# xuekt98/BBDM

Measured on NVIDIA H100. Metric: denoising-steps/sec (UNet fwd) at 256^2 pixel-BBDM, higher is better.
Workload: dtype bf16x3 (split-bf16 tensor-core products, fp32 accumulate: fp32-class)

## Files before the change

### bbdm_b200/csrc/conv_umma.cu

```cuda
#include "tc_common.cuh"
#include <stdlib.h>

namespace bbdm {

constexpr int UM_BM = 128;
constexpr int UM_BK = 64;
constexpr int UM_THREADS = 384;
constexpr int UM_PRODUCER_REGS = 40, UM_CONSUMER_REGS = 232;
static_assert(128 * UM_PRODUCER_REGS + 256 * UM_CONSUMER_REGS <= 65536, "conv_umma: register split");
constexpr int UM_SLICES = 4;

struct ConvParams {
  int B, H, W, Cout;
  int TW, TH, TB, tiles_w, tiles_h, tiles_b, n_tiles;
  int kb_per_tap;
  int K1;
  int K2;
  int taps;
  int up2;
  int origin;
  int w_per_image;
  int kb_per_chunk;
  const float* bias; const float* bias2;
  const float* residual; int res_mode;
  float* out; __nv_bfloat16* out_hi; __nv_bfloat16* out_lo;
  int out_nchw_c;
  float* stats;
  unsigned long long* fault;
};

template <int BN>
struct UmmaCfg {
  static constexpr uint32_t A_BYTES = UM_BM * UM_BK * 2;
  static constexpr uint32_t W_BYTES = BN * UM_BK * 2;
  static constexpr uint32_t STAGE3 = 2 * A_BYTES + 2 * W_BYTES;
  static constexpr uint32_t STAGE1 = A_BYTES + W_BYTES;
  static constexpr uint32_t SMEM_BUDGET = 200 * 1024;
  static constexpr int STAGES3 = (SMEM_BUDGET / STAGE3) > 6 ? 6 : (SMEM_BUDGET / STAGE3);
  static constexpr int STAGES1 = (SMEM_BUDGET / STAGE1) > 8 ? 8 : (SMEM_BUDGET / STAGE1);
};

template <int BN, bool F16>
__device__ __forceinline__ void conv_mma(float* d, uint64_t da, uint64_t db) {
  if (F16) {
    if (BN == 128) wgmma_n128_f16<0>(d, da, db, 1u); else wgmma_n64_f16<0>(d, da, db, 1u);
  } else {
    if (BN == 128) wgmma_n128_bf16<0>(d, da, db, 1u); else wgmma_n64_bf16<0>(d, da, db, 1u);
  }
}

struct EpiTile {
  int nb, tw, th, tb, phase;
  int bb[2], hh[2], ww[2];
  bool valid[2];
  int64_t pix[2];
};

__device__ __forceinline__ EpiTile epi_tile(const ConvParams& p, int tile, int n_blocks, int warp, int lane) {
  EpiTile e;
  e.nb = tile % n_blocks;
  int mt = tile / n_blocks;
  e.phase = 0;
  if (p.up2) { e.phase = mt & 3; mt >>= 2; }
  e.tw = mt % p.tiles_w; mt /= p.tiles_w;
  e.th = mt % p.tiles_h;
  e.tb = mt / p.tiles_h;
  const int OH = p.up2 ? 2 * p.H : p.H, OW = p.up2 ? 2 * p.W : p.W;
#pragma unroll
  for (int ri = 0; ri < 2; ++ri) {
    const int row = 16 * warp + (lane >> 2) + 8 * ri;
    const int ws = e.tw * p.TW + row % p.TW;
    const int hs = e.th * p.TH + (row / p.TW) % p.TH;
    e.bb[ri] = e.tb * p.TB + row / (p.TW * p.TH);
    e.valid[ri] = ws < p.W && hs < p.H && e.bb[ri] < p.B;
    e.hh[ri] = p.up2 ? 2 * hs + (e.phase >> 1) : hs;
    e.ww[ri] = p.up2 ? 2 * ws + (e.phase & 1) : ws;
    e.pix[ri] = ((int64_t)e.bb[ri] * OH + e.hh[ri]) * OW + e.ww[ri];
  }
  return e;
}

template <int BN>
__device__ __forceinline__ void epi_slice(const ConvParams& p, const float* racc, EpiTile e, int s, int warp,
                                          int lane, float (*stats_s)[BN][2]) {
  constexpr int JS = BN / 8 / UM_SLICES;
  if (e.nb * BN + s * (BN / UM_SLICES) >= p.Cout) return;
  asm volatile("" : "+r"(e.nb), "+r"(e.bb[0]), "+r"(e.bb[1]), "+r"(e.hh[0]), "+r"(e.hh[1]), "+r"(e.ww[0]),
               "+r"(e.ww[1]), "+l"(e.pix[0]), "+l"(e.pix[1]));
  const int OH = p.up2 ? 2 * p.H : p.H, OW = p.up2 ? 2 * p.W : p.W;
  const int n0 = e.nb * BN + 2 * (lane & 3);
  float2 v[2][JS];
#pragma unroll
  for (int ri = 0; ri < 2; ++ri) {
#pragma unroll
    for (int j = 0; j < JS; ++j) {
      const int jj = JS * s + j;
      const int nc = n0 + 8 * jj;
      v[ri][j] = make_float2(racc[4 * jj + 2 * ri], racc[4 * jj + 2 * ri + 1]);
      if (p.bias) { const float2 b = *reinterpret_cast<const float2*>(p.bias + nc); v[ri][j].x += b.x; v[ri][j].y += b.y; }
      if (p.bias2) { const float2 b = *reinterpret_cast<const float2*>(p.bias2 + nc); v[ri][j].x += b.x; v[ri][j].y += b.y; }
    }
  }
  if (p.res_mode == BBDM_RES_SAME || p.res_mode == BBDM_RES_UP2) {
#pragma unroll
    for (int ri = 0; ri < 2; ++ri) {
      if (!e.valid[ri]) continue;
      const int64_t rpix = p.res_mode == BBDM_RES_SAME
                               ? e.pix[ri]
                               : ((int64_t)e.bb[ri] * (OH >> 1) + (e.hh[ri] >> 1)) * (OW >> 1) + (e.ww[ri] >> 1);
      const float* rp = p.residual + rpix * p.Cout + n0 + 8 * JS * s;
#pragma unroll
      for (int j = 0; j < JS; ++j) {
        const float2 t = *reinterpret_cast<const float2*>(rp + 8 * j);
        v[ri][j].x += t.x; v[ri][j].y += t.y;
      }
    }
  } else if (p.res_mode == BBDM_RES_DOWN2) {
    const int64_t W2 = (int64_t)OW * 2;
#pragma unroll
    for (int ri = 0; ri < 2; ++ri) {
      if (!e.valid[ri]) continue;
      const float* rp0 = p.residual + (((int64_t)e.bb[ri] * OH * 2 + e.hh[ri] * 2) * W2 + e.ww[ri] * 2) * p.Cout +
                         n0 + 8 * JS * s;
#pragma unroll
      for (int j = 0; j < JS; ++j) {
        const float* rp = rp0 + 8 * j;
        const float2 t0 = *reinterpret_cast<const float2*>(rp), t1 = *reinterpret_cast<const float2*>(rp + p.Cout);
        const float2 t2 = *reinterpret_cast<const float2*>(rp + W2 * p.Cout);
        const float2 t3 = *reinterpret_cast<const float2*>(rp + (W2 + 1) * p.Cout);
        v[ri][j].x += 0.25f * (((t0.x + t1.x) + t2.x) + t3.x);
        v[ri][j].y += 0.25f * (((t0.y + t1.y) + t2.y) + t3.y);
      }
    }
  }
  float ssum[2 * JS], ssq[2 * JS];
#pragma unroll
  for (int j = 0; j < 2 * JS; ++j) { ssum[j] = 0.f; ssq[j] = 0.f; }
#pragma unroll
  for (int ri = 0; ri < 2; ++ri) {
    if (!e.valid[ri]) continue;
    const int bb = e.bb[ri], hh = e.hh[ri], ww = e.ww[ri];
    const int64_t pix = e.pix[ri];
#pragma unroll
    for (int j = 0; j < JS; ++j) {
      const int nc = n0 + 8 * (JS * s + j);
      const float2 w = v[ri][j];
      if (p.out_nchw_c > 0) {
        if (nc < p.out_nchw_c) p.out[(((int64_t)bb * p.out_nchw_c + nc) * OH + hh) * OW + ww] = w.x;
        if (nc + 1 < p.out_nchw_c) p.out[(((int64_t)bb * p.out_nchw_c + nc + 1) * OH + hh) * OW + ww] = w.y;
      } else if (p.out) {
        *reinterpret_cast<float2*>(p.out + pix * p.Cout + nc) = w;
      }
      if (p.out_hi) {
        uint32_t h, l;
        split2x(w.x, w.y, h, l);
        *reinterpret_cast<uint32_t*>(p.out_hi + pix * p.Cout + nc) = h;
        *reinterpret_cast<uint32_t*>(p.out_lo + pix * p.Cout + nc) = l;
      }
      ssum[2 * j] += w.x; ssq[2 * j] += w.x * w.x;
      ssum[2 * j + 1] += w.y; ssq[2 * j + 1] += w.y * w.y;
    }
  }
  if (p.stats) {
#pragma unroll
    for (int j = 0; j < 2 * JS; ++j) {
#pragma unroll
      for (int off = 4; off < 32; off <<= 1) {
        ssum[j] += __shfl_xor_sync(0xffffffffu, ssum[j], off);
        ssq[j] += __shfl_xor_sync(0xffffffffu, ssq[j], off);
      }
    }
    if (lane < 4) {
#pragma unroll
      for (int j = 0; j < 2 * JS; ++j) {
        const int c = 8 * (JS * s + (j >> 1)) + 2 * lane + (j & 1);
        stats_s[warp][c][0] = ssum[j];
        stats_s[warp][c][1] = ssq[j];
      }
    }
  }
}

template <int BN>
__device__ __forceinline__ void epi_stats_out(const ConvParams& p, const EpiTile& e, float (*stats_s)[BN][2]) {
  if (!p.stats) return;
  asm volatile("bar.sync 1, 256;" ::: "memory");
  const int64_t tile_lin =
      (((int64_t)e.tb * p.tiles_w * p.tiles_h + e.th * p.tiles_w + e.tw) * (p.up2 ? 4 : 1) + e.phase) * 4;
  int i0 = threadIdx.x;
  asm volatile("" : "+r"(i0));
  for (int i = i0; i < 4 * BN; i += 256) {
    const int q = i / BN, c = i % BN;
    if (e.nb * BN + c >= p.Cout) continue;
    const float s = stats_s[2 * q][c][0] + stats_s[2 * q + 1][c][0];
    const float sq = stats_s[2 * q][c][1] + stats_s[2 * q + 1][c][1];
    *reinterpret_cast<float2*>(p.stats + ((tile_lin + q) * p.Cout + e.nb * BN + c) * 2) = make_float2(s, sq);
  }
  asm volatile("bar.sync 1, 256;" ::: "memory");
}

template <int BN>
__device__ __forceinline__ void epi_slices(const ConvParams& p, const float* racc, const EpiTile& e, int s_begin,
                                           int s_end, int warp, int lane, float (*stats_s)[BN][2]) {
#pragma unroll
  for (int s = 0; s < UM_SLICES; ++s)
    if (s >= s_begin && s < s_end) epi_slice<BN>(p, racc, e, s, warp, lane, stats_s);
}

template <int BN, int PASSES, bool F16>
__global__ void __launch_bounds__(UM_THREADS, 1)
conv_umma_kernel(const __grid_constant__ CUtensorMap map_a_hi, const __grid_constant__ CUtensorMap map_a_lo,
                 const __grid_constant__ CUtensorMap map_w_hi, const __grid_constant__ CUtensorMap map_w_lo,
                 const __grid_constant__ CUtensorMap map_a2_hi, const __grid_constant__ CUtensorMap map_a2_lo,
                 const __grid_constant__ CUtensorMap map_w2_hi, const __grid_constant__ CUtensorMap map_w2_lo,
                 const ConvParams p) {
  using Cfg = UmmaCfg<BN>;
  constexpr int STAGES = PASSES == 3 ? Cfg::STAGES3 : Cfg::STAGES1;
  constexpr uint32_t STAGE_BYTES = PASSES == 3 ? Cfg::STAGE3 : Cfg::STAGE1;
  constexpr uint32_t OFF_ALO = Cfg::A_BYTES;
  constexpr uint32_t OFF_WHI = PASSES == 3 ? 2 * Cfg::A_BYTES : Cfg::A_BYTES;
  constexpr uint32_t OFF_WLO = OFF_WHI + Cfg::W_BYTES;
  constexpr int NR = BN / 2;
  static_assert(STAGES >= 2, "need at least a double buffer");

  extern __shared__ uint8_t smem_raw[];
  __shared__ __align__(8) uint64_t bars[2 * 8];
  __shared__ int abort_s;
  __shared__ __align__(16) float stats_s[8][BN][2];

  const uint32_t tiles_base = (smem_u32(smem_raw) + 1023u) & ~1023u;
  const int warp = threadIdx.x >> 5, lane = threadIdx.x & 31;
  const uint32_t bar_full = smem_u32(&bars[0]);
  const uint32_t bar_empty = smem_u32(&bars[8]);
  volatile int* abort_flag = &abort_s;

  if (threadIdx.x == 0) {
    abort_s = 0;
    for (int i = 0; i < STAGES; ++i) { mbar_init(bar_full + 8 * i, 1); mbar_init(bar_empty + 8 * i, 8); }
    asm volatile("fence.mbarrier_init.release.cluster;" ::: "memory");
  }
  __syncthreads();

  const int n_blocks = (p.Cout + BN - 1) / BN;
  const int total_tiles = p.n_tiles * n_blocks * (p.up2 ? 4 : 1);
  const int KB = p.K1 + p.K2;

  if (warp >= 8) {
    setmaxnreg_dec<UM_PRODUCER_REGS>();
    if (warp == 8 && lane == 0) {
      int stage = 0;
      uint32_t phase_bit = 0;
      for (int tile = blockIdx.x; tile < total_tiles; tile += gridDim.x) {
        const int nb = tile % n_blocks;
        int mt = tile / n_blocks;
        int phase = 0;
        if (p.up2) { phase = mt & 3; mt >>= 2; }
        const int tw = mt % p.tiles_w; mt /= p.tiles_w;
        const int th = mt % p.tiles_h;
        const int tb = mt / p.tiles_h;
        const int w0 = tw * p.TW, h0 = th * p.TH, b0 = tb * p.TB, n0 = nb * BN;
        for (int kb = 0; kb < KB; ++kb) {
          mbar_wait(bar_empty + 8 * stage, phase_bit ^ 1, abort_flag, p.fault, 0xE0000000ull | (unsigned)kb);
          const uint32_t sbase = tiles_base + stage * STAGE_BYTES;
          const uint32_t full = bar_full + 8 * stage;
          mbar_expect_tx(full, STAGE_BYTES);
          if (kb < p.K1) {
            const int tap = kb / p.kb_per_tap, cb = kb - tap * p.kb_per_tap;
            int dy = 0, dx = 0, wtap = tap;
            if (p.up2) {
              const int r = tap >> 1, c = tap & 1;
              dy = (phase >> 1) ? r : r - 1;
              dx = (phase & 1) ? c : c - 1;
              wtap = phase * 4 + tap;
            } else if (p.taps == 9) { dy = tap / 3 - 1; dx = tap % 3 - 1; }
            else if (p.taps == 4) { dy = (tap >> 1) + p.origin; dx = (tap & 1) + p.origin; }
            else if (p.w_per_image) wtap = tb;
            tma_load_4d(sbase, &map_a_hi, full, cb * UM_BK, w0 + dx, h0 + dy, b0);
            if (PASSES == 3) tma_load_4d(sbase + OFF_ALO, &map_a_lo, full, cb * UM_BK, w0 + dx, h0 + dy, b0);
            tma_load_3d(sbase + OFF_WHI, &map_w_hi, full, cb * UM_BK, n0, wtap);
            if (PASSES == 3) tma_load_3d(sbase + OFF_WLO, &map_w_lo, full, cb * UM_BK, n0, wtap);
          } else {
            const int cb = kb - p.K1;
            tma_load_4d(sbase, &map_a2_hi, full, cb * UM_BK, w0, h0, b0);
            if (PASSES == 3) tma_load_4d(sbase + OFF_ALO, &map_a2_lo, full, cb * UM_BK, w0, h0, b0);
            tma_load_3d(sbase + OFF_WHI, &map_w2_hi, full, cb * UM_BK, n0, 0);
            if (PASSES == 3) tma_load_3d(sbase + OFF_WLO, &map_w2_lo, full, cb * UM_BK, n0, 0);
          }
          if (++stage == STAGES) { stage = 0; phase_bit ^= 1; }
        }
      }
    }
    return;
  }

  setmaxnreg_inc<UM_CONSUMER_REGS>();
  const int wg = warp >> 2;
  const uint32_t a_off = (uint32_t)wg * 64 * 128;
  int stage = 0;
  uint32_t phase_bit = 0;
  float racc[NR];
  EpiTile pend;
  bool pending = false;
  int slice = 0;
  for (int tile = blockIdx.x; tile < total_tiles; tile += gridDim.x) {
    for (int kb0 = 0; kb0 < KB; kb0 += p.kb_per_chunk) {
      const int kb1 = kb0 + p.kb_per_chunk < KB ? kb0 + p.kb_per_chunk : KB;
      float acc[NR];
#pragma unroll
      for (int j = 0; j < NR; ++j) acc[j] = 0.f;
      int prev = -1;
      for (int kb = kb0; kb < kb1; ++kb) {
        mbar_wait(bar_full + 8 * stage, phase_bit, abort_flag, p.fault, 0xF0000000ull | (unsigned)kb);
        const uint32_t sbase = tiles_base + stage * STAGE_BYTES;
        const uint64_t da_hi = make_sw128_desc(sbase + a_off);
        const uint64_t da_lo = make_sw128_desc(sbase + OFF_ALO + a_off);
        const uint64_t db_hi = make_sw128_desc(sbase + OFF_WHI);
        const uint64_t db_lo = make_sw128_desc(sbase + OFF_WLO);
        wgmma_fence();
#pragma unroll
        for (int k = 0; k < UM_BK / 16; ++k) {
          const uint64_t ko = (uint64_t)(k * 32 >> 4);
          if (PASSES == 3) {
            conv_mma<BN, F16>(acc, da_lo + ko, db_hi + ko);
            conv_mma<BN, F16>(acc, da_hi + ko, db_lo + ko);
          }
          conv_mma<BN, F16>(acc, da_hi + ko, db_hi + ko);
        }
        wgmma_commit();
        wgmma_wait<1>();
        if (prev >= 0 && lane == 0) mbar_arrive(bar_empty + 8 * prev);
        prev = stage;
        if (++stage == STAGES) { stage = 0; phase_bit ^= 1; }
        if (pending) {
          const int s_end = kb + 1 < kb1 ? slice + 1 : UM_SLICES;
          epi_slices<BN>(p, racc, pend, slice, s_end, warp, lane, stats_s);
          slice = s_end;
        }
      }
      if (pending) {
        epi_stats_out<BN>(p, pend, stats_s);
        pending = false;
      }
      wgmma_wait<0>();
      reg_fence<NR>(acc);
      if (lane == 0) mbar_arrive(bar_empty + 8 * prev);
      if (kb0 == 0) {
#pragma unroll
        for (int j = 0; j < NR; ++j) racc[j] = 0.f + acc[j];
      } else {
#pragma unroll
        for (int j = 0; j < NR; ++j) racc[j] += acc[j];
      }
    }
    pend = epi_tile(p, tile, n_blocks, warp, lane);
    pending = true;
    slice = 0;
  }
  if (pending) {
    epi_slices<BN>(p, racc, pend, 0, UM_SLICES, warp, lane, stats_s);
    epi_stats_out<BN>(p, pend, stats_s);
  }
}

static int make_act_map(CUtensorMap* m, const void* ptr, int B, int H, int W, int C, int TW, int TH, int TB,
                        bool f16) {
  EncodeTiledFn enc = get_encode();
  BBDM_REQUIRE(enc != nullptr, "cuTensorMapEncodeTiled entry point not available");
  cuuint64_t dims[4] = {(cuuint64_t)C, (cuuint64_t)W, (cuuint64_t)H, (cuuint64_t)B};
  cuuint64_t strides[3] = {(cuuint64_t)C * 2, (cuuint64_t)W * C * 2, (cuuint64_t)H * W * C * 2};
  cuuint32_t box[4] = {(cuuint32_t)UM_BK, (cuuint32_t)TW, (cuuint32_t)TH, (cuuint32_t)TB};
  cuuint32_t es[4] = {1, 1, 1, 1};
  CUresult r = enc(m, f16 ? CU_TENSOR_MAP_DATA_TYPE_FLOAT16 : CU_TENSOR_MAP_DATA_TYPE_BFLOAT16, 4, const_cast<void*>(ptr), dims, strides, box, es,
                   CU_TENSOR_MAP_INTERLEAVE_NONE, CU_TENSOR_MAP_SWIZZLE_128B, CU_TENSOR_MAP_L2_PROMOTION_L2_256B,
                   CU_TENSOR_MAP_FLOAT_OOB_FILL_NONE);
  BBDM_REQUIRE(r == CUDA_SUCCESS, "cuTensorMapEncodeTiled(activation) failed: %d (B=%d H=%d W=%d C=%d box=%dx%dx%d)",
               (int)r, B, H, W, C, TW, TH, TB);
  return BBDM_OK;
}

static int make_w_map(CUtensorMap* m, const void* ptr, int taps, int Cout, int Cin, int BN, bool f16) {
  EncodeTiledFn enc = get_encode();
  BBDM_REQUIRE(enc != nullptr, "cuTensorMapEncodeTiled entry point not available");
  cuuint64_t dims[3] = {(cuuint64_t)Cin, (cuuint64_t)Cout, (cuuint64_t)taps};
  cuuint64_t strides[2] = {(cuuint64_t)Cin * 2, (cuuint64_t)Cout * Cin * 2};
  cuuint32_t box[3] = {(cuuint32_t)UM_BK, (cuuint32_t)BN, 1};
  cuuint32_t es[3] = {1, 1, 1};
  CUresult r = enc(m, f16 ? CU_TENSOR_MAP_DATA_TYPE_FLOAT16 : CU_TENSOR_MAP_DATA_TYPE_BFLOAT16, 3, const_cast<void*>(ptr), dims, strides, box, es,
                   CU_TENSOR_MAP_INTERLEAVE_NONE, CU_TENSOR_MAP_SWIZZLE_128B, CU_TENSOR_MAP_L2_PROMOTION_L2_256B,
                   CU_TENSOR_MAP_FLOAT_OOB_FILL_NONE);
  BBDM_REQUIRE(r == CUDA_SUCCESS, "cuTensorMapEncodeTiled(weight) failed: %d (taps=%d Cout=%d Cin=%d BN=%d)", (int)r,
               taps, Cout, Cin, BN);
  return BBDM_OK;
}

static int pow2_floor(int x) { int p = 1; while (p * 2 <= x) p *= 2; return p; }
static int pow2_ceil(int x) { int p = 1; while (p < x) p *= 2; return p; }

template <int BN, int PASSES, bool F16>
static int launch_conv(const CUtensorMap* maps, const ConvParams& p, int grid, cudaStream_t s) {
  using Cfg = UmmaCfg<BN>;
  constexpr int STAGES = PASSES == 3 ? Cfg::STAGES3 : Cfg::STAGES1;
  constexpr uint32_t STAGE_BYTES = PASSES == 3 ? Cfg::STAGE3 : Cfg::STAGE1;
  const size_t smem = (size_t)STAGES * STAGE_BYTES + 1024;
  static DeviceOnce configured;
  if (configured.need()) {
    BBDM_CUDA_CHECK(cudaFuncSetAttribute(conv_umma_kernel<BN, PASSES, F16>, cudaFuncAttributeMaxDynamicSharedMemorySize, (int)smem));
    configured.mark();
  }
  conv_umma_kernel<BN, PASSES, F16><<<grid, UM_THREADS, smem, s>>>(maps[0], maps[1], maps[2], maps[3], maps[4], maps[5],
                                                                  maps[6], maps[7], p);
  BBDM_LAUNCH_CHECK();
  return BBDM_OK;
}

}

using namespace bbdm;

static void tile_geometry(int H, int W, int* TW, int* TH, int* TB) {
  *TW = pow2_floor(W) < 16 ? pow2_floor(W) : 16;
  const int th = pow2_ceil(H);
  *TH = th < UM_BM / *TW ? th : UM_BM / *TW;
  *TB = UM_BM / (*TW * *TH);
}

extern "C" int bbdm_conv_umma_geometry(int H, int W, int* TW, int* TH, int* TB, int* rows_per_image) {
  BBDM_REQUIRE(H > 0 && W >= 4, "conv_umma_geometry: need H > 0, W >= 4");
  int tw, th, tb;
  tile_geometry(H, W, &tw, &th, &tb);
  if (TW) *TW = tw;
  if (TH) *TH = th;
  if (TB) *TB = tb;
  if (rows_per_image) *rows_per_image = tb == 1 ? 4 * ((W + tw - 1) / tw) * ((H + th - 1) / th) : 0;
  return BBDM_OK;
}

extern "C" int bbdm_conv_umma(const BbdmConvArgs* a, void* stream) {
  BBDM_REQUIRE(a != nullptr, "conv_umma: null args");
  BBDM_REQUIRE(a->B > 0 && a->H > 0 && a->W > 0, "conv_umma: bad spatial shape");
  BBDM_REQUIRE(a->taps == 1 || a->taps == 9 || a->taps == 4, "conv_umma: taps must be 1, 4 or 9 (got %d)", a->taps);
  BBDM_REQUIRE(!a->upsample2x || (a->taps == 4 && a->Cin2 == 0), "conv_umma: upsample2x needs the 16 phase taps and no fused 1x1");
  BBDM_REQUIRE(a->Cin > 0 && a->Cin % 32 == 0, "conv_umma: Cin %% 32 != 0 (Cin=%d)", a->Cin);
  BBDM_REQUIRE(a->Cout > 0 && a->Cout % 32 == 0, "conv_umma: Cout %% 32 != 0 (Cout=%d)", a->Cout);
  BBDM_REQUIRE(a->Cin2 >= 0 && a->Cin2 % 32 == 0, "conv_umma: Cin2 %% 32 != 0 (Cin2=%d)", a->Cin2);
  BBDM_REQUIRE(a->passes == 1 || a->passes == 3, "conv_umma: passes must be 1 or 3");
  BBDM_REQUIRE(a->a_hi && a->w_hi && (a->passes == 1 || (a->a_lo && a->w_lo)), "conv_umma: missing operand plane");
  if (a->Cin2) BBDM_REQUIRE(a->a2_hi && a->w2_hi && (a->passes == 1 || (a->a2_lo && a->w2_lo)), "conv_umma: missing 1x1 operand plane");
  BBDM_REQUIRE(a->out || (a->out_hi && a->out_lo), "conv_umma: no output");
  BBDM_REQUIRE((a->out_hi == nullptr) == (a->out_lo == nullptr), "conv_umma: out hi/lo must come in pairs");
  BBDM_REQUIRE(a->res_mode >= 0 && a->res_mode <= 3 && (a->res_mode == 0 || a->residual), "conv_umma: bad residual");
  if (a->res_mode == BBDM_RES_UP2 && !a->upsample2x) BBDM_REQUIRE(a->H % 2 == 0 && a->W % 2 == 0, "conv_umma: RES_UP2 needs even H, W");
  BBDM_REQUIRE(a->W >= 4, "conv_umma: W < 4 not supported (use conv_direct)");
  BBDM_REQUIRE(a->window_origin == 0 || a->window_origin == -1, "conv_umma: window_origin must be 0 or -1 (got %d)",
               a->window_origin);
  BBDM_REQUIRE(a->window_origin == 0 || (a->taps == 4 && !a->upsample2x),
               "conv_umma: window_origin -1 needs taps == 4 and no upsample2x");
  const bool wpi = a->weights_per_image != 0, f16 = a->operand_f16 != 0;
  if (wpi) BBDM_REQUIRE(a->taps == 1 && a->Cin2 == 0 && !a->upsample2x, "conv_umma: weights_per_image needs taps == 1 and no fused operand");
  if (wpi) BBDM_REQUIRE(a->Cin % 64 == 0 && a->Cout % 64 == 0, "conv_umma: weights_per_image needs Cin, Cout %% 64 == 0");

  ConvParams p;
  p.B = a->B; p.H = a->H; p.W = a->W; p.Cout = a->Cout;
  tile_geometry(a->H, a->W, &p.TW, &p.TH, &p.TB);
  p.tiles_w = (a->W + p.TW - 1) / p.TW;
  p.tiles_h = (a->H + p.TH - 1) / p.TH;
  p.tiles_b = (a->B + p.TB - 1) / p.TB;
  p.n_tiles = p.tiles_w * p.tiles_h * p.tiles_b;
  int BN = (a->Cout + 127) / 128 * 128 == (a->Cout + 63) / 64 * 64 ? 128 : 64;
  {
    const int64_t m_tiles = (int64_t)p.n_tiles * (a->upsample2x ? 4 : 1);
    const int64_t want = (int64_t)(0.7 * num_sms());
    if (BN > 64 && m_tiles * ((a->Cout + BN - 1) / BN) < want) BN = 64;
  }
  p.kb_per_tap = (a->Cin + UM_BK - 1) / UM_BK;
  p.K1 = a->taps * p.kb_per_tap;
  p.K2 = (a->Cin2 + UM_BK - 1) / UM_BK;
  p.taps = a->taps;
  p.up2 = a->upsample2x ? 1 : 0;
  p.origin = a->window_origin;
  p.w_per_image = wpi ? 1 : 0;
  static int wino_chunk = -1;
  if (wino_chunk < 0) { const char* e = getenv("BBDM_WINO_CHUNK"); wino_chunk = (e && atoi(e) > 0) ? atoi(e) : 0; }
  const int wchunk = wino_chunk ? wino_chunk : (a->Cin >= 512 ? 4 : 2);
  p.kb_per_chunk = wpi ? wchunk : (a->passes == 3 ? 4 : 8);
  if (wpi) BBDM_REQUIRE(p.TB == 1, "conv_umma: weights_per_image needs 128-pixel tiles inside one image (H*W >= 128)");
  p.bias = a->bias; p.bias2 = a->Cin2 ? a->bias2 : nullptr;
  p.residual = a->residual; p.res_mode = a->res_mode;
  p.out = a->out; p.out_hi = (__nv_bfloat16*)a->out_hi; p.out_lo = (__nv_bfloat16*)a->out_lo;
  p.out_nchw_c = a->out_nchw_channels;
  p.stats = a->stats_partial;
  BBDM_REQUIRE(p.out_nchw_c >= 0 && p.out_nchw_c <= a->Cout && (p.out_nchw_c == 0 || (a->out && !a->out_hi)),
               "conv_umma: bad out_nchw_channels");
  p.fault = device_fault_ptr();
  BBDM_REQUIRE(p.fault != nullptr, "conv_umma: device fault word unavailable");

  BBDM_REQUIRE(p.stats == nullptr || (p.TB == 1 && p.out_nchw_c == 0),
               "conv_umma: stats_partial needs a tile inside one image (H*W >= 128) and NHWC output");
  CUtensorMap maps[8];
  int rc;
  if ((rc = make_act_map(&maps[0], a->a_hi, a->B, a->H, a->W, a->Cin, p.TW, p.TH, p.TB, f16))) return rc;
  if ((rc = make_act_map(&maps[1], a->passes == 3 ? a->a_lo : a->a_hi, a->B, a->H, a->W, a->Cin, p.TW, p.TH, p.TB, f16))) return rc;
  const int wtaps = a->upsample2x ? 16 : (wpi ? a->B : a->taps);
  if ((rc = make_w_map(&maps[2], a->w_hi, wtaps, a->Cout, a->Cin, BN, f16))) return rc;
  if ((rc = make_w_map(&maps[3], a->passes == 3 ? a->w_lo : a->w_hi, wtaps, a->Cout, a->Cin, BN, f16))) return rc;
  if (a->Cin2) {
    if ((rc = make_act_map(&maps[4], a->a2_hi, a->B, a->H, a->W, a->Cin2, p.TW, p.TH, p.TB, f16))) return rc;
    if ((rc = make_act_map(&maps[5], a->passes == 3 ? a->a2_lo : a->a2_hi, a->B, a->H, a->W, a->Cin2, p.TW, p.TH, p.TB, f16))) return rc;
    if ((rc = make_w_map(&maps[6], a->w2_hi, 1, a->Cout, a->Cin2, BN, f16))) return rc;
    if ((rc = make_w_map(&maps[7], a->passes == 3 ? a->w2_lo : a->w2_hi, 1, a->Cout, a->Cin2, BN, f16))) return rc;
  } else {
    maps[4] = maps[0]; maps[5] = maps[1]; maps[6] = maps[2]; maps[7] = maps[3];
  }
  const int64_t total = (int64_t)p.n_tiles * ((a->Cout + BN - 1) / BN) * (p.up2 ? 4 : 1);
  BBDM_REQUIRE(total < (1ll << 30), "conv_umma: too many tiles");
  const int grid = (int)(total < num_sms() ? total : num_sms());
  cudaStream_t s = (cudaStream_t)stream;
  const bool p3 = a->passes == 3;
  if (BN == 128) {
    if (f16) return p3 ? launch_conv<128, 3, true>(maps, p, grid, s) : launch_conv<128, 1, true>(maps, p, grid, s);
    return p3 ? launch_conv<128, 3, false>(maps, p, grid, s) : launch_conv<128, 1, false>(maps, p, grid, s);
  }
  if (f16) return p3 ? launch_conv<64, 3, true>(maps, p, grid, s) : launch_conv<64, 1, true>(maps, p, grid, s);
  return p3 ? launch_conv<64, 3, false>(maps, p, grid, s) : launch_conv<64, 1, false>(maps, p, grid, s);
}
```

Baseline: 6.071.

## Add specialized wgmma GEMM kernel for per-image-weight Winograd batched products

Adds a dedicated warp-specialized TMA+wgmma kernel for the per-image-weight (Winograd-style batched) GEMM case with no residual, stats, or split outputs. It ping-pongs two accumulator sets so that folding one chunk's partial sums overlaps with the next chunk's async MMAs, and it uses a simplified epilogue. The aim is to shed the generic conv kernel's epilogue and slice overhead on this path. The cost is extra register pressure from holding three accumulator arrays and one more kernel variant to maintain.

```diff
diff --git a/bbdm_b200/csrc/conv_umma.cu b/bbdm_b200/csrc/conv_umma.cu
--- a/bbdm_b200/csrc/conv_umma.cu
+++ b/bbdm_b200/csrc/conv_umma.cu
@@ -362,6 +362,199 @@
   }
 }
 
+
+template <int BN, bool F16>
+__device__ __forceinline__ void wino_mma(float* d, uint64_t da, uint64_t db, uint32_t scale_d) {
+  if (F16) {
+    if (BN == 128) wgmma_n128_f16<0>(d, da, db, scale_d); else wgmma_n64_f16<0>(d, da, db, scale_d);
+  } else {
+    if (BN == 128) wgmma_n128_bf16<0>(d, da, db, scale_d); else wgmma_n64_bf16<0>(d, da, db, scale_d);
+  }
+}
+
+template <int BN>
+__device__ __forceinline__ void wino_store(const ConvParams& p, const float* racc, int tile, int n_blocks, int warp,
+                                           int lane) {
+  const int nb = tile % n_blocks;
+  int mt = tile / n_blocks;
+  const int tw = mt % p.tiles_w; mt /= p.tiles_w;
+  const int th = mt % p.tiles_h;
+  const int tb = mt / p.tiles_h;
+  const int n0 = nb * BN + 2 * (lane & 3);
+#pragma unroll
+  for (int ri = 0; ri < 2; ++ri) {
+    const int row = 16 * warp + (lane >> 2) + 8 * ri;
+    const int ws = tw * p.TW + row % p.TW, hs = th * p.TH + row / p.TW;
+    if (ws >= p.W || hs >= p.H) continue;
+    float* op = p.out + (((int64_t)tb * p.H + hs) * p.W + ws) * p.Cout + n0;
+#pragma unroll
+    for (int jj = 0; jj < BN / 8; ++jj) {
+      float2 v = make_float2(racc[4 * jj + 2 * ri], racc[4 * jj + 2 * ri + 1]);
+      if (p.bias) { const float2 b = *reinterpret_cast<const float2*>(p.bias + n0 + 8 * jj); v.x += b.x; v.y += b.y; }
+      *reinterpret_cast<float2*>(op + 8 * jj) = v;
+    }
+  }
+}
+
+struct WinoStream {
+  int tile, kb0, stage, prev, pend_tile;
+  uint32_t phase_bit;
+  bool pend, pend_first, pend_last;
+};
+
+template <int BN>
+__device__ __forceinline__ void wino_fold(const ConvParams& p, WinoStream& s, float* racc, float* acc, int n_blocks,
+                                          int warp, int lane) {
+  constexpr int NR = BN / 2;
+  reg_fence<NR>(acc);
+  if (s.pend_first) {
+#pragma unroll
+    for (int j = 0; j < NR; ++j) racc[j] = 0.f + acc[j];
+  } else {
+#pragma unroll
+    for (int j = 0; j < NR; ++j) racc[j] += acc[j];
+  }
+  if (s.pend_last) wino_store<BN>(p, racc, s.pend_tile, n_blocks, warp, lane);
+  s.pend = false;
+}
+
+template <int BN, int PASSES, bool F16, uint32_t STAGE_BYTES, int STAGES>
+__device__ __forceinline__ bool wino_chunk(const ConvParams& p, WinoStream& s, float* racc, float* acc, float* other,
+                                           uint32_t tiles_base, uint32_t bar_full, uint32_t bar_empty,
+                                           volatile int* abort_flag, int total_tiles, int n_blocks, int KB, int warp,
+                                           int lane) {
+  constexpr int NR = BN / 2;
+  constexpr uint32_t OFF_ALO = UmmaCfg<BN>::A_BYTES;
+  constexpr uint32_t OFF_WHI = PASSES == 3 ? 2 * UmmaCfg<BN>::A_BYTES : UmmaCfg<BN>::A_BYTES;
+  constexpr uint32_t OFF_WLO = OFF_WHI + UmmaCfg<BN>::W_BYTES;
+  if (s.tile >= total_tiles) return false;
+  const uint32_t a_off = (uint32_t)(warp >> 2) * 64 * 128;
+  const int kb1 = s.kb0 + p.kb_per_chunk < KB ? s.kb0 + p.kb_per_chunk : KB;
+  for (int kb = s.kb0; kb < kb1; ++kb) {
+    mbar_wait(bar_full + 8 * s.stage, s.phase_bit, abort_flag, p.fault, 0xF6000000ull | (unsigned)kb);
+    const uint32_t sbase = tiles_base + s.stage * STAGE_BYTES;
+    const uint64_t da_hi = make_sw128_desc(sbase + a_off);
+    const uint64_t da_lo = make_sw128_desc(sbase + OFF_ALO + a_off);
+    const uint64_t db_hi = make_sw128_desc(sbase + OFF_WHI);
+    const uint64_t db_lo = make_sw128_desc(sbase + OFF_WLO);
+    wgmma_fence();
+#pragma unroll
+    for (int k = 0; k < UM_BK / 16; ++k) {
+      const uint64_t ko = (uint64_t)(k * 32 >> 4);
+      const uint32_t keep = (k == 0 && kb == s.kb0) ? 0u : 1u;
+      if (PASSES == 3) {
+        wino_mma<BN, F16>(acc, da_lo + ko, db_hi + ko, keep);
+        wino_mma<BN, F16>(acc, da_hi + ko, db_lo + ko, 1u);
+      }
+      wino_mma<BN, F16>(acc, da_hi + ko, db_hi + ko, PASSES == 3 ? 1u : keep);
+    }
+    wgmma_commit();
+    wgmma_wait<1>();
+    if (s.prev >= 0 && lane == 0) mbar_arrive(bar_empty + 8 * s.prev);
+    s.prev = s.stage;
+    if (++s.stage == STAGES) { s.stage = 0; s.phase_bit ^= 1; }
+    if (s.pend) wino_fold<BN>(p, s, racc, other, n_blocks, warp, lane);
+  }
+  s.pend = true;
+  s.pend_tile = s.tile;
+  s.pend_first = s.kb0 == 0;
+  s.pend_last = kb1 == KB;
+  s.kb0 = kb1;
+  if (s.kb0 == KB) { s.kb0 = 0; s.tile += gridDim.x; }
+  return true;
+}
+
+template <int BN, int PASSES, bool F16>
+__device__ __forceinline__ void wino_drain(const ConvParams& p, WinoStream& s, float* racc, float* acc,
+                                           uint32_t bar_empty, int n_blocks, int warp, int lane) {
+  if (!s.pend) return;
+  wgmma_wait<0>();
+  if (lane == 0) mbar_arrive(bar_empty + 8 * s.prev);
+  wino_fold<BN>(p, s, racc, acc, n_blocks, warp, lane);
+}
+
+template <int BN, int PASSES, bool F16>
+__global__ void __launch_bounds__(UM_THREADS, 1)
+wino_gemm_kernel(const __grid_constant__ CUtensorMap map_a_hi, const __grid_constant__ CUtensorMap map_a_lo,
+                 const __grid_constant__ CUtensorMap map_w_hi, const __grid_constant__ CUtensorMap map_w_lo,
+                 const ConvParams p) {
+  using Cfg = UmmaCfg<BN>;
+  constexpr int STAGES = PASSES == 3 ? Cfg::STAGES3 : Cfg::STAGES1;
+  constexpr uint32_t STAGE_BYTES = PASSES == 3 ? Cfg::STAGE3 : Cfg::STAGE1;
+  constexpr uint32_t OFF_ALO = Cfg::A_BYTES;
+  constexpr uint32_t OFF_WHI = PASSES == 3 ? 2 * Cfg::A_BYTES : Cfg::A_BYTES;
+  constexpr uint32_t OFF_WLO = OFF_WHI + Cfg::W_BYTES;
+  constexpr int NR = BN / 2;
+  static_assert(STAGES >= 2, "need at least a double buffer");
+
+  extern __shared__ uint8_t smem_raw[];
+  __shared__ __align__(8) uint64_t bars[2 * 8];
+  __shared__ int abort_s;
+
+  const uint32_t tiles_base = (smem_u32(smem_raw) + 1023u) & ~1023u;
+  const int warp = threadIdx.x >> 5, lane = threadIdx.x & 31;
+  const uint32_t bar_full = smem_u32(&bars[0]);
+  const uint32_t bar_empty = smem_u32(&bars[8]);
+  volatile int* abort_flag = &abort_s;
+
+  if (threadIdx.x == 0) {
+    abort_s = 0;
+    for (int i = 0; i < STAGES; ++i) { mbar_init(bar_full + 8 * i, 1); mbar_init(bar_empty + 8 * i, 8); }
+    asm volatile("fence.mbarrier_init.release.cluster;" ::: "memory");
+  }
+  __syncthreads();
+
+  const int n_blocks = p.Cout / BN;
+  const int total_tiles = p.n_tiles * n_blocks;
+  const int KB = p.K1;
+
+  if (warp >= 8) {
+    setmaxnreg_dec<UM_PRODUCER_REGS>();
+    if (warp == 8 && lane == 0) {
+      int stage = 0;
+      uint32_t phase_bit = 0;
+      for (int tile = blockIdx.x; tile < total_tiles; tile += gridDim.x) {
+        const int nb = tile % n_blocks;
+        int mt = tile / n_blocks;
+        const int tw = mt % p.tiles_w; mt /= p.tiles_w;
+        const int th = mt % p.tiles_h;
+        const int tb = mt / p.tiles_h;
+        const int w0 = tw * p.TW, h0 = th * p.TH, n0 = nb * BN;
+        for (int kb = 0; kb < KB; ++kb) {
+          mbar_wait(bar_empty + 8 * stage, phase_bit ^ 1, abort_flag, p.fault, 0xE6000000ull | (unsigned)kb);
+          const uint32_t sbase = tiles_base + stage * STAGE_BYTES;
+          const uint32_t full = bar_full + 8 * stage;
+          mbar_expect_tx(full, STAGE_BYTES);
+          tma_load_4d(sbase, &map_a_hi, full, kb * UM_BK, w0, h0, tb);
+          if (PASSES == 3) tma_load_4d(sbase + OFF_ALO, &map_a_lo, full, kb * UM_BK, w0, h0, tb);
+          tma_load_3d(sbase + OFF_WHI, &map_w_hi, full, kb * UM_BK, n0, tb);
+          if (PASSES == 3) tma_load_3d(sbase + OFF_WLO, &map_w_lo, full, kb * UM_BK, n0, tb);
+          if (++stage == STAGES) { stage = 0; phase_bit ^= 1; }
+        }
+      }
+    }
+    return;
+  }
+
+  setmaxnreg_inc<UM_CONSUMER_REGS>();
+  float racc[NR], acc0[NR], acc1[NR];
+  WinoStream s;
+  s.tile = blockIdx.x; s.kb0 = 0; s.stage = 0; s.prev = -1; s.pend_tile = -1; s.phase_bit = 0;
+  s.pend = s.pend_first = s.pend_last = false;
+  for (;;) {
+    if (!wino_chunk<BN, PASSES, F16, STAGE_BYTES, STAGES>(p, s, racc, acc0, acc1, tiles_base, bar_full, bar_empty,
+                                                          abort_flag, total_tiles, n_blocks, KB, warp, lane)) {
+      wino_drain<BN, PASSES, F16>(p, s, racc, acc1, bar_empty, n_blocks, warp, lane);
+      break;
+    }
+    if (!wino_chunk<BN, PASSES, F16, STAGE_BYTES, STAGES>(p, s, racc, acc1, acc0, tiles_base, bar_full, bar_empty,
+                                                          abort_flag, total_tiles, n_blocks, KB, warp, lane)) {
+      wino_drain<BN, PASSES, F16>(p, s, racc, acc0, bar_empty, n_blocks, warp, lane);
+      break;
+    }
+  }
+}
+
 static int make_act_map(CUtensorMap* m, const void* ptr, int B, int H, int W, int C, int TW, int TH, int TB,
                         bool f16) {
   EncodeTiledFn enc = get_encode();
@@ -409,6 +602,22 @@
   }
   conv_umma_kernel<BN, PASSES, F16><<<grid, UM_THREADS, smem, s>>>(maps[0], maps[1], maps[2], maps[3], maps[4], maps[5],
                                                                   maps[6], maps[7], p);
+  BBDM_LAUNCH_CHECK();
+  return BBDM_OK;
+}
+
+template <int BN, int PASSES, bool F16>
+static int launch_wino(const CUtensorMap* maps, const ConvParams& p, int grid, cudaStream_t s) {
+  using Cfg = UmmaCfg<BN>;
+  constexpr int STAGES = PASSES == 3 ? Cfg::STAGES3 : Cfg::STAGES1;
+  constexpr uint32_t STAGE_BYTES = PASSES == 3 ? Cfg::STAGE3 : Cfg::STAGE1;
+  const size_t smem = (size_t)STAGES * STAGE_BYTES + 1024;
+  static DeviceOnce configured;
+  if (configured.need()) {
+    BBDM_CUDA_CHECK(cudaFuncSetAttribute(wino_gemm_kernel<BN, PASSES, F16>, cudaFuncAttributeMaxDynamicSharedMemorySize, (int)smem));
+    configured.mark();
+  }
+  wino_gemm_kernel<BN, PASSES, F16><<<grid, UM_THREADS, smem, s>>>(maps[0], maps[1], maps[2], maps[3], p);
   BBDM_LAUNCH_CHECK();
   return BBDM_OK;
 }
@@ -516,6 +725,14 @@
   const int grid = (int)(total < num_sms() ? total : num_sms());
   cudaStream_t s = (cudaStream_t)stream;
   const bool p3 = a->passes == 3;
+  if (wpi && p.res_mode == BBDM_RES_NONE && !p.stats && !p.out_hi && !p.out_nchw_c && p.out) {
+    if (BN == 128) {
+      if (f16) return p3 ? launch_wino<128, 3, true>(maps, p, grid, s) : launch_wino<128, 1, true>(maps, p, grid, s);
+      return p3 ? launch_wino<128, 3, false>(maps, p, grid, s) : launch_wino<128, 1, false>(maps, p, grid, s);
+    }
+    if (f16) return p3 ? launch_wino<64, 3, true>(maps, p, grid, s) : launch_wino<64, 1, true>(maps, p, grid, s);
+    return p3 ? launch_wino<64, 3, false>(maps, p, grid, s) : launch_wino<64, 1, false>(maps, p, grid, s);
+  }
   if (BN == 128) {
     if (f16) return p3 ? launch_conv<128, 3, true>(maps, p, grid, s) : launch_conv<128, 1, true>(maps, p, grid, s);
     return p3 ? launch_conv<128, 3, false>(maps, p, grid, s) : launch_conv<128, 1, false>(maps, p, grid, s);
```

New measurement: 6.599 (median of 6 runs). +8.7%, better.
